# lalithsuresh/rapid

Hardware: NVIDIA H100
Metric: alert_cells_per_sec_to_converged_cut (higher is better)
Workload: dtype u16

## Files before the change

rapid_b200/csrc/cd_bucketed.cu:

```cuda
#include <cooperative_groups.h>

#include <algorithm>
#include <climits>
#include <cstdlib>

#include "cd_internal.cuh"

namespace cg = cooperative_groups;

namespace rapid {

constexpr int UNI_MINBLOCKS = 5;
constexpr int PF_DIST = 2;

constexpr int TILE_R = 1024;
constexpr int UNI_THREADS = 128;
constexpr int GEN_THREADS = 256;
constexpr int STAGE = 32;
constexpr int MAXK = RAPID_MAX_K;
constexpr int SMALL_SEG = 4;
constexpr uint32_t T32_NONE = 0xFFFFFFFFu;
constexpr uint64_t T64_NONE = ~0ULL;
constexpr uint32_t RF_K3 = 16u;
constexpr uint32_t RF_ACTIVE = 32u;
constexpr uint32_t RF_MIXED_EMIT = 64u;

constexpr uint32_t MX_ON = 1u, MX_NEG = 2u, MX_HAS_E = 4u, MX_DONE = 8u;
constexpr uint32_t MX_REF = 32u;
constexpr uint32_t MX_TIME = 16u;

constexpr uint32_t PF_SEEN = 1u;
constexpr uint32_t PF_NEGINF = 2u;

struct ChunkAcc {
    uint32_t nL, nH, tp, nUn, fl, minTH, minTLun, pad_;
    uint64_t h1, h2;
    uint32_t nLp, nHp, tpc, minBHp, minBLlong, pad2_;
    uint64_t h1p, h2p;
};

constexpr int PF_SHIFT = 30;
constexpr uint32_t TP_MASK = (1u << PF_SHIFT) - 1u;

struct Partials {
    uint4* cnt;
    uint4* cntp;
    uint64_t* minTH;
    uint64_t* minTLun;
    uint64_t* h1;
    uint64_t* h2;
    uint64_t* h1p;
    uint64_t* h2p;
    uint2* seq;
    int32_t* flag;
    ChunkAcc* chunk;
    int n_tiles;
};

struct Bucketed {
    DevBuf<int32_t> sidx;
    DevBuf<int32_t> seg_cnt, batch_slots;
    DevBuf<int32_t> bins, ovf, cell_batch;
    DevBuf<SubjDesc> desc;
    DevBuf<SubjWalk> walk;
    DevBuf<uint8_t> s_ring, s_status;
    DevBuf<int32_t> p_flag;
    DevBuf<ChunkAcc> p_chunk;
    DevBuf<uint4> p_cnt, p_cntp;
    DevBuf<uint64_t> p_minTH, p_minTLun, p_h1, p_h2, p_h1p, p_h2p;
    DevBuf<uint2> p_seq;
    DevBuf<SubjWalk> pwalk;
    DevBuf<unsigned char> ra_dev;
    DevBuf<uint32_t> mx_fl;
    DevBuf<uint64_t> mx_a, mx_cand, mx_emax;
    DevBuf<uint64_t> mx_p1, mx_p2;
    DevBuf<int32_t> mx_pc;
    DevBuf<unsigned long long> mx_e1, mx_e2;
    DevBuf<int32_t> mx_ec;
    DevBuf<uint64_t> estar;
    DevBuf<int32_t> mx_changed;
    DevBuf<uint32_t> mx_dev;
    DevBuf<int32_t> batch_index;
    DevBuf<int32_t> inv_res, inv_ticket;
    DevBuf<unsigned long long> inv_h1, inv_h2;
    DevBuf<int32_t> wl_slots, wl_count, wl_listed, wl_so_tab;
    DevBuf<uint8_t> wl_in_tile;
    DevBuf<uint8_t> has_so;
    size_t in_list_slots = 0;
    int n_tiles = 0;
    size_t part_cap = 0;
    int slots_uniform = 0, slots_generic = 0;
    int resolve_grid = 0;
};

struct Visit {
    int c0, c1;
    bool crossL, crossH;
    uint32_t tL, tH;
};

__device__ __forceinline__ Visit visit_uniform(uint32_t ur, const SubjDesc& d, const SubjWalk& w, int L, int H) {
    Visit v;
    v.tL = 0; v.tH = 0;
    if (ur == d.pmask) {
        v.c0 = __popc(ur); v.c1 = __popc(ur | d.bmask);
        v.tL = d.tLf; v.tH = d.tHf;
    } else {
        int c = __popc(ur);
        v.c0 = c;
        const int nr = d.nr;
        for (int q = 0; q < nr; ++q) {
            const int k = w.ring[q];
            const bool isnew = !((ur >> k) & 1u);
            c += isnew;
            if (isnew && c == L) v.tL = w.time[q];
            if (isnew && c == H) v.tH = w.time[q];
        }
        v.c1 = c;
    }
    v.crossL = v.c0 < L && v.c1 >= L;
    v.crossH = v.c0 < H && v.c1 >= H;
    return v;
}

__device__ __forceinline__ Visit visit_counts(uint32_t ur, const SubjDesc& d, uint32_t RM, int L, int H) {
    Visit v;
    v.tL = 0; v.tH = 0;
    v.c0 = __popc(ur);
    v.c1 = __popc((ur | d.bmask) & RM);
    v.crossL = v.c0 < L && v.c1 >= L;
    v.crossH = v.c0 < H && v.c1 >= H;
    return v;
}

struct Acc {
    uint32_t nL = 0, nH = 0, tp = 0, nUn = 0, flags = 0;
    uint32_t minTH = T32_NONE, minTLun = T32_NONE;
    uint64_t h1 = 0, h2 = 0;
    uint32_t nLp = 0, nHp = 0, tpc = 0, minBHp = T32_NONE, minBLlong = T32_NONE;
    uint64_t h1p = 0, h2p = 0;
};

__device__ __forceinline__ bool accumulate(Acc& a, const Visit& v, const SubjDesc& d, int L, int H) {
    if (v.c0 >= L && v.c0 < H) a.tp++;
    if (v.crossL) a.nL++;
    if (v.crossH) { a.nH++; a.minTH = min(a.minTH, v.tH); a.h1 += d.mix1; a.h2 += d.mix2; }
    if (v.c1 >= L && v.c1 < H) {
        if (v.crossL) { a.nUn++; a.minTLun = min(a.minTLun, v.tL); }
        else a.flags |= PF_NEGINF;
        return true;
    }
    return false;
}

__device__ __forceinline__ uint32_t prefix_core(Acc* acc, uint32_t ur, const SubjDesc& d, const SubjWalk& pw, const uint32_t* u,
                                                uint32_t umask, int L, int H, uint32_t last) {
    const int c0 = __popc(ur);
    int c = c0;
    uint32_t word = ur, bLp = 0, bHp = 0;
    if (ur == 0 && umask == 0) {
        c = __popc(d.pmask); bLp = d.f_bLp; bHp = d.f_bHp; word = d.pmask;
    } else {
        const int np = __popc(d.pmask);
        uint32_t imp = umask & ~ur;
        uint32_t bL = c >= L ? 0u : T32_NONE;
        int q = 0;
        for (;;) {
            while (q < np && ((word >> pw.ring[q]) & 1u)) ++q;
            const uint32_t te = q < np ? pw.time[q] : T32_NONE;
            uint32_t ti = T32_NONE;
            if (imp && c >= L && c < H) {
                for (uint32_t m = imp; m; m &= m - 1) { const int k = __ffs(m) - 1; if (u[k] != T32_NONE) ti = min(ti, max(u[k], bL)); }
                if (ti > last) ti = T32_NONE;
            }
            if (ti != T32_NONE && ti < te) {
                for (uint32_t m = imp; m; m &= m - 1) {
                    const int k = __ffs(m) - 1;
                    if (u[k] == T32_NONE || u[k] > ti) continue;
                    word |= 1u << k; imp &= ~(1u << k);
                    ++c;
                    if (c == H) bHp = ti;
                }
                if (c >= H) imp = 0;
            } else if (te != T32_NONE) {
                const int k = pw.ring[q];
                word |= 1u << k; imp &= ~(1u << k);
                ++c; ++q;
                if (c == L) { bL = te; bLp = te; }
                if (c == H) bHp = te;
            } else {
                break;
            }
        }
    }
    if (acc) {
        if (c0 >= L && c0 < H) acc->tpc++;
        if (c0 < L && c >= L) acc->nLp++;
        if (c0 < H && c >= H) { acc->nHp++; acc->h1p += d.mix1; acc->h2p += d.mix2; acc->minBHp = min(acc->minBHp, bHp); }
        if (c >= L && c < H) acc->minBLlong = min(acc->minBLlong, c0 >= L ? 0u : bLp);
    }
    return word;
}

__device__ __forceinline__ uint32_t observer_L_batch(uint32_t uo, const SubjDesc* dobs, const SubjWalk* pwo, int L) {
    int c = __popc(uo);
    if (c >= L) return 0u;
    if (dobs == nullptr || dobs->pmask == 0) return T32_NONE;
    const int np = __popc(dobs->pmask);
    for (int q = 0; q < np; ++q) {
        if ((uo >> pwo->ring[q]) & 1u) continue;
        if (++c == L) return pwo->time[q];
    }
    return T32_NONE;
}

struct ApplyArgs {
    RowRef rows;
    size_t Rpad;
    int K, H, L;
    int64_t R, rbegin;
    const uint32_t* rflags;
    DeliveryDev dl;
    const BatchCounts* bc;
    const SubjDesc* desc;
    const SubjWalk* walk;
    const SubjWalk* pwalk;
    const int32_t* touch;
    const int32_t* batch_index;
    int32_t serial;
    int seq;
    const int32_t* slot_subject;
    const int32_t* sidx;
    const uint8_t* s_ring;
    const uint8_t* s_status;
    Partials part;
    int n_tiles;
    WorkList wl;
};

__device__ __forceinline__ void note_unresolved(const ApplyArgs& a, int tile, int32_t slot) { worklist_note(a.wl, tile, slot); }

template <bool SEQ>
__device__ __forceinline__ void part_store(const Partials& p, size_t at, const Acc& a) {
    p.cnt[at] = make_uint4(a.nL, a.nH, a.tp | (a.flags << PF_SHIFT), a.nUn);
    if (SEQ) p.cntp[at] = make_uint4(a.nLp, a.nHp, a.tpc, 0u);
    p.minTH[at] = a.minTH == T32_NONE ? T64_NONE : (uint64_t)a.minTH;
    p.minTLun[at] = a.minTLun == T32_NONE ? T64_NONE : (uint64_t)a.minTLun;
    p.h1[at] = a.h1;
    p.h2[at] = a.h2;
    if (SEQ) { p.h1p[at] = a.h1p; p.h2p[at] = a.h2p; p.seq[at] = make_uint2(a.minBHp, a.minBLlong); }
}
template <bool SEQ>
__device__ __forceinline__ void part_merge(const Partials& p, size_t at, const Acc& a) {
    uint4 c = p.cnt[at];
    c.x += a.nL; c.y += a.nH; c.z = (c.z + a.tp) | (a.flags << PF_SHIFT); c.w += a.nUn;
    p.cnt[at] = c;
    if (SEQ && (a.nLp | a.nHp | a.tpc)) { uint4 cp = p.cntp[at]; cp.x += a.nLp; cp.y += a.nHp; cp.z += a.tpc; p.cntp[at] = cp; }
    if (a.minTH != T32_NONE) { const uint64_t o = p.minTH[at]; if ((uint64_t)a.minTH < o) p.minTH[at] = a.minTH; }
    if (a.minTLun != T32_NONE) { const uint64_t o = p.minTLun[at]; if ((uint64_t)a.minTLun < o) p.minTLun[at] = a.minTLun; }
    if (a.nH) { p.h1[at] += a.h1; p.h2[at] += a.h2; }
    if (SEQ) {
        if (a.nHp) { p.h1p[at] += a.h1p; p.h2p[at] += a.h2p; }
        uint2 q = p.seq[at];
        q.x = min(q.x, a.minBHp); q.y = min(q.y, a.minBLlong);
        p.seq[at] = q;
    }
}

struct StageAcc {
    uint32_t nLH, tpUn, fl, minTH, minTLun;
    uint64_t h1, h2;
    uint32_t nLHp, tpc, minBHp, minBLlong;
    uint64_t h1p, h2p;
};

template <bool SEQ>
__device__ __forceinline__ StageAcc stage_pack(const Acc& f) {
    StageAcc s;
    s.nLH = f.nL | (f.nH << 16); s.tpUn = f.tp | (f.nUn << 16); s.fl = f.flags; s.minTH = f.minTH; s.minTLun = f.minTLun;
    s.h1 = f.h1; s.h2 = f.h2;
    s.nLHp = SEQ ? f.nLp | (f.nHp << 16) : 0u; s.tpc = SEQ ? f.tpc : 0u; s.minBHp = SEQ ? f.minBHp : T32_NONE;
    s.minBLlong = SEQ ? f.minBLlong : T32_NONE; s.h1p = SEQ ? f.h1p : 0ull; s.h2p = SEQ ? f.h2p : 0ull;
    return s;
}
template <bool SEQ>
__device__ __forceinline__ StageAcc stage_reduce(StageAcc s) {
#pragma unroll
    for (int o = 16; o > 0; o >>= 1) {
        s.nLH += __shfl_down_sync(0xffffffffu, s.nLH, o);
        s.tpUn += __shfl_down_sync(0xffffffffu, s.tpUn, o);
        s.fl |= __shfl_down_sync(0xffffffffu, s.fl, o);
        s.minTH = min(s.minTH, __shfl_down_sync(0xffffffffu, s.minTH, o));
        s.minTLun = min(s.minTLun, __shfl_down_sync(0xffffffffu, s.minTLun, o));
        s.h1 += __shfl_down_sync(0xffffffffu, s.h1, o);
        s.h2 += __shfl_down_sync(0xffffffffu, s.h2, o);
        if (SEQ) {
            s.nLHp += __shfl_down_sync(0xffffffffu, s.nLHp, o);
            s.tpc += __shfl_down_sync(0xffffffffu, s.tpc, o);
            s.minBHp = min(s.minBHp, __shfl_down_sync(0xffffffffu, s.minBHp, o));
            s.minBLlong = min(s.minBLlong, __shfl_down_sync(0xffffffffu, s.minBLlong, o));
            s.h1p += __shfl_down_sync(0xffffffffu, s.h1p, o);
            s.h2p += __shfl_down_sync(0xffffffffu, s.h2p, o);
        }
    }
    return s;
}
template <bool SEQ>
__device__ __forceinline__ void chunk_add(ChunkAcc& c, const StageAcc& m) {
    c.nL += m.nLH & 0xFFFFu; c.nH += m.nLH >> 16; c.tp += m.tpUn & 0xFFFFu; c.nUn += m.tpUn >> 16; c.fl |= m.fl;
    c.minTH = min(c.minTH, m.minTH); c.minTLun = min(c.minTLun, m.minTLun); c.h1 += m.h1; c.h2 += m.h2;
    if (SEQ) {
        c.nLp += m.nLHp & 0xFFFFu; c.nHp += m.nLHp >> 16; c.tpc += m.tpc; c.minBHp = min(c.minBHp, m.minBHp);
        c.minBLlong = min(c.minBLlong, m.minBLlong); c.h1p += m.h1p; c.h2p += m.h2p;
    }
}
__device__ __forceinline__ ChunkAcc chunk_zero() {
    ChunkAcc c;
    c.nL = 0; c.nH = 0; c.tp = 0; c.nUn = 0; c.fl = 0; c.minTH = T32_NONE; c.minTLun = T32_NONE; c.pad_ = 0; c.h1 = 0; c.h2 = 0;
    c.nLp = 0; c.nHp = 0; c.tpc = 0; c.minBHp = T32_NONE; c.minBLlong = T32_NONE; c.pad2_ = 0; c.h1p = 0; c.h2p = 0;
    return c;
}
template <bool SEQ>
__device__ __forceinline__ void acc_add(Acc& a, const StageAcc& m) {
    a.nL += m.nLH & 0xFFFFu; a.nH += m.nLH >> 16; a.tp += m.tpUn & 0xFFFFu; a.nUn += m.tpUn >> 16; a.flags |= m.fl;
    a.minTH = min(a.minTH, m.minTH); a.minTLun = min(a.minTLun, m.minTLun); a.h1 += m.h1; a.h2 += m.h2;
    if (SEQ) {
        a.nLp += m.nLHp & 0xFFFFu; a.nHp += m.nLHp >> 16; a.tpc += m.tpc; a.minBHp = min(a.minBHp, m.minBHp);
        a.minBLlong = min(a.minBLlong, m.minBLlong); a.h1p += m.h1p; a.h2p += m.h2p;
    }
}

template <bool PERM, bool SEQ>
__device__ __forceinline__ bool visit_acc(Acc& acc, uint32_t ur, const SubjDesc& d, const SubjWalk* w, const SubjWalk* pw, uint32_t RM, int L, int H,
                                          const uint32_t* u = nullptr, uint32_t umask = 0, uint32_t last = 0, uint32_t* word_out = nullptr) {
    if (SEQ) ur = prefix_core(&acc, ur, d, *pw, u, umask, L, H, last);
    if (word_out) *word_out = ur;
    const Visit v = PERM ? visit_counts(ur & RM, d, RM, L, H) : visit_uniform(ur & RM, d, *w, L, H);
    return accumulate(acc, v, d, L, H);
}

constexpr uint32_t RF_PRE_DOWN = 128u;
__device__ __forceinline__ uint32_t receiver_down_batch(const ApplyArgs& a, uint32_t rflag, bool after_finalize1) {
    if (rflag & (after_finalize1 ? RF_PRE_DOWN : RF_SEEN_DOWN)) return 0u;
    const int32_t sd = a.bc->seq_down;
    return sd == INT_MAX ? T32_NONE : (uint32_t)sd;
}
__device__ __forceinline__ const uint8_t* precall_row(const ApplyArgs& a, int32_t slot, bool post_flip) {
    const int flipped = post_flip && a.touch[slot] == a.serial ? 1 : 0;
    return a.rows.lo(slot, a.rows.cur[slot] ^ flipped);
}
__device__ __noinline__ uint32_t edge_times(const ApplyArgs& a, int32_t slot, int64_t r, bool post_flip, uint32_t bDown, uint32_t* u) {
    if (!a.wl.has_so[slot]) return 0u;
    const uint32_t RM = (1u << a.K) - 1u;
    const int32_t S_before = a.bc->S_before;
    uint32_t umask = 0;
    for (int k = 0; k < a.K; ++k) {
        const int32_t so = a.wl.so_tab[(size_t)slot * SO_STRIDE + k];
        if (so < 0) continue;
        const bool ot = a.touch[so] == a.serial;
        const int bo = ot ? a.batch_index[so] : 0;
        const uint32_t uo = so >= S_before ? 0u : (a.rows.get(precall_row(a, so, post_flip), r) & RM);
        const uint32_t bLo = observer_L_batch(uo, ot ? &a.desc[bo] : nullptr, ot ? &a.pwalk[bo] : nullptr, a.L);
        u[k] = (bLo == T32_NONE || bDown == T32_NONE) ? T32_NONE : max(bLo, bDown);
        umask |= 1u << k;
    }
    return umask;
}
__device__ __forceinline__ uint32_t seq_state(const ApplyArgs& a, const SubjDesc& d, int b_index, int64_t r, uint32_t old, bool post_flip,
                                              bool after_finalize1) {
    if (!a.seq) return old;
    uint32_t u[MAXK];
    const uint32_t umask = edge_times(a, d.slot, r, post_flip, receiver_down_batch(a, a.rflags[r], after_finalize1), u);
    if (umask == 0 && d.pmask == 0) return old;
    return prefix_core(nullptr, old, d, a.pwalk[b_index], u, umask, a.L, a.H, (uint32_t)a.bc->seq_last);
}

template <bool PERM, bool SEQ, int HB>
__global__ void __launch_bounds__(UNI_THREADS, UNI_MINBLOCKS) k_apply_uniform(const ApplyArgs a) {
    __shared__ SubjDesc sd[STAGE];
    __shared__ SubjWalk sw[PERM ? 1 : STAGE];
    __shared__ SubjWalk spw[SEQ ? STAGE : 1];
    __shared__ const uint8_t* s_src[STAGE];
    __shared__ uint8_t* s_dst[STAGE];
    __shared__ uint32_t s_nw[STAGE];
    __shared__ uint2 s_nrep[STAGE];
    __shared__ int s_unres[STAGE];
    __shared__ ChunkAcc s_facc;
    __shared__ int s_heavy;
    __shared__ uint8_t s_ne[SEQ ? STAGE : 1];
    __shared__ uint8_t s_ek[SEQ ? STAGE : 1][MAXK];
    __shared__ const uint8_t* s_erow[SEQ ? STAGE : 1][MAXK];
    __shared__ int32_t s_eob[SEQ ? STAGE : 1][MAXK];
    __shared__ uint32_t s_mst[STAGE];
    __shared__ uint2 s_mrep[STAGE];
    __shared__ uint8_t s_mun[STAGE];
    __shared__ StageAcc s_macc[STAGE];
    __shared__ StageAcc s_msum;
    __shared__ uint32_t s_mall;
    __shared__ int s_wfirst[UNI_THREADS / 32];

    constexpr bool MEMO = !SEQ;
    if (a.bc->overflow) return;
    const int Sb = a.bc->n_batch_subj, S_before = a.bc->S_before;
    const int per_chunk = max(1, (Sb + (int)gridDim.y - 1) / (int)gridDim.y);
    const int tile = blockIdx.x, chunk = blockIdx.y, t = threadIdx.x;
    const int s0 = min(Sb, chunk * per_chunk), s1 = min(Sb, s0 + per_chunk);
    const int64_t r0 = (int64_t)tile * TILE_R + (int64_t)t * 8;
    const size_t pbase = (size_t)chunk * a.Rpad + (size_t)r0;
    const uint32_t RM = (1u << a.K) - 1u;
    const int L = a.L, H = a.H;
    const uint32_t seq_last = SEQ ? (uint32_t)a.bc->seq_last : 0u;

    uint32_t act = 0, seen = 0;
#pragma unroll
    for (int j = 0; j < 8; ++j) {
        const int64_t r = r0 + j;
        if (r < a.R) {
            const uint32_t rf = a.rflags[r];
            const bool on = !(rf & RF_ANNOUNCED) && !((a.dl.flags & RAPID_DELIVERY_BLOCKED) && a.dl.blocked[r]);
            act |= (on ? 1u : 0u) << j;
            if (SEQ && (rf & RF_SEEN_DOWN)) seen |= 1u << j;
        }
    }
    const Group8<HB> am = group8_mask<HB>(act);
    const RowRef& rows = a.rows;
    if (t == 0) s_facc = chunk_zero();
    if (MEMO) {
        const int mine = act ? t * 8 + __ffs(act) - 1 : INT_MAX;
        const int wmin = __reduce_min_sync(0xffffffffu, mine);
        if ((t & 31) == 0) s_wfirst[t >> 5] = wmin;
    }
    const int block_active = __syncthreads_or(act != 0);
    int sample_r = 0;
    if (MEMO && t < 32) {
        int f = INT_MAX;
#pragma unroll
        for (int q = 0; q < UNI_THREADS / 32; ++q) f = min(f, s_wfirst[q]);
        sample_r = f == INT_MAX ? 0 : f;
    }
    const size_t sample_at = (size_t)tile * TILE_R + (size_t)sample_r;
    Acc com;
    bool had_exc = false;
    bool carried = false;

    for (int base = s0; base < s1; base += STAGE) {
        const int n = min(STAGE, s1 - base);
        __syncthreads();
        if (t < 32) {
            Acc f;
            Acc m;
            bool heavy = false, memo = false;
            if (t < n) {
                const SubjDesc d = a.desc[base + t];
                sd[t] = d;
                const uint8_t c = rows.cur[d.slot];
                const bool fresh = d.slot >= S_before;
                s_src[t] = fresh ? nullptr : rows.lo(d.slot, c);
                s_dst[t] = rows.lo(d.slot, c ^ 1);
                s_nw[t] = (uint32_t)(d.bmask | d.pmask);
                s_nrep[t] = group8_rep<HB>(d.bmask | d.pmask);
                int un = 0;
                const bool edges = SEQ && a.wl.has_so[d.slot];
                if (SEQ) {
                    int ne = 0;
                    if (edges) {
                        for (int k = 0; k < a.K; ++k) {
                            const int32_t so = a.wl.so_tab[(size_t)d.slot * SO_STRIDE + k];
                            if (so < 0) continue;
                            s_ek[t][ne] = (uint8_t)k;
                            s_erow[t][ne] = so >= S_before ? nullptr : rows.cur_lo(so);
                            s_eob[t][ne] = a.touch[so] == a.serial ? a.batch_index[so] : -1;
                            ++ne;
                        }
                    }
                    s_ne[t] = (uint8_t)ne;
                }
                if (fresh && !edges) {
                    un = (visit_acc<PERM, SEQ>(f, 0u, d, &sw[0], &spw[0], RM, L, H) && block_active) ? 1 : 0;
                    if (PERM) { f.minTH = T32_NONE; f.minTLun = T32_NONE; }
                } else {
                    if (!PERM) sw[t] = a.walk[base + t];
                    if (SEQ) spw[t] = a.pwalk[base + t];
                    if (fresh) s_src[t] = nullptr;
                    if (MEMO && !fresh && !edges && block_active) {
                        const uint32_t sst = rows.get(s_src[t], (int64_t)sample_at);
                        uint32_t at_last = sst;
                        const bool mun = visit_acc<PERM, SEQ>(m, sst & RM, d, &sw[PERM ? 0 : t], &spw[SEQ ? t : 0], RM, L, H, nullptr, 0u, seq_last, &at_last);
                        s_mst[t] = sst;
                        s_mrep[t] = group8_rep<HB>((SEQ ? at_last : sst) | s_nw[t]);
                        s_mun[t] = mun ? 1 : 0;
                        memo = true;
                    }
                }
                if (MEMO) { if (!memo) s_mst[t] = 0xFFFFFFFFu; else s_macc[t] = stage_pack<SEQ>(m); }
                s_unres[t] = (un && a.wl.has_so[d.slot]) ? 1 : 0;
                if (!fresh || edges) s_unres[t] = a.wl.has_so[d.slot] ? 0 : -1;
                heavy = !fresh || edges;
            }
            {
                const unsigned hm = __ballot_sync(0xffffffffu, heavy);
                if (t == 0) s_heavy = __popc(hm);
            }
            const StageAcc fr = stage_reduce<SEQ>(stage_pack<SEQ>(f));
            if (t == 0) chunk_add<SEQ>(s_facc, fr);
            if (MEMO) {
                const unsigned mm = __ballot_sync(0xffffffffu, memo);
                if (mm) {
                    const StageAcc mr = stage_reduce<SEQ>(stage_pack<SEQ>(m));
                    if (t == 0) s_msum = mr;
                }
                if (t == 0) s_mall = mm;
            }
        }
        __syncthreads();
        uint32_t hit = 0;
        const bool pf_on = !SEQ && s_heavy != 0;
        if (pf_on) {
#pragma unroll
            for (int j = 0; j < PF_DIST; ++j)
                if (j < n && s_src[j]) {
                    asm volatile("prefetch.global.L2 [%0];" ::"l"(s_src[j] + r0));
                    asm volatile("prefetch.global.L2 [%0];" ::"l"(group8_hi<HB>(rows, s_src[j], r0)));
                }
        }
#pragma unroll 4
        for (int i = 0; i < n; ++i) {
            const uint8_t* src = s_src[i];
            uint8_t* dst = s_dst[i];
            const int ne = SEQ ? (int)s_ne[i] : 0;
            if (pf_on && i + PF_DIST < n) {
                const uint8_t* nx = s_src[i + PF_DIST];
                if (nx) {
                    asm volatile("prefetch.global.L2 [%0];" ::"l"(nx + r0));
                    asm volatile("prefetch.global.L2 [%0];" ::"l"(group8_hi<HB>(rows, nx, r0)));
                }
            }
            if (src == nullptr && ne == 0) {
                group8_store<HB>(rows, dst, r0, group8_fill<HB>(s_nrep[i], am));
                continue;
            }
            Group8<HB> w;
            if (src) w = group8_load<HB>(rows, src, r0);
            else { w.lo = 0; w.hi = 0; }
            bool unres = false;
            if (act) {
                const SubjDesc& d = sd[i];
                uint32_t st;
                bool same = group8_same<HB>(w, am, &st);
                carried = true;
                const bool mhit = MEMO && same && st == s_mst[i];
                uint32_t u[MAXK];
                uint32_t umask = 0;
                if (SEQ && ne && !mhit) {
                    const uint32_t sact = seen & act;
                    same = same && (sact == 0 || sact == act);
                    const uint32_t bDown = sact ? 0u : (a.bc->seq_down == INT_MAX ? T32_NONE : (uint32_t)a.bc->seq_down);
                    for (int e = 0; e < ne && same; ++e) {
                        uint32_t so_st = 0;
                        if (s_erow[i][e]) same = group8_same<HB>(group8_load<HB>(rows, s_erow[i][e], r0), am, &so_st);
                        const int ob = s_eob[i][e], k = s_ek[i][e];
                        const uint32_t bLo = observer_L_batch(so_st & RM, ob >= 0 ? &a.desc[ob] : nullptr, ob >= 0 ? &a.pwalk[ob] : nullptr, L);
                        u[k] = (bLo == T32_NONE || bDown == T32_NONE) ? T32_NONE : max(bLo, bDown);
                        umask |= 1u << k;
                    }
                }
                if (mhit) {
                    hit |= 1u << i;
                    unres = s_mun[i] != 0;
                    group8_merge<HB>(w, s_mrep[i], am);
                } else if (same) {
                    uint32_t at_last = st;
                    unres = visit_acc<PERM, SEQ>(com, st & RM, d, &sw[PERM ? 0 : i], &spw[SEQ ? i : 0], RM, L, H, u, umask, seq_last, &at_last);
                    group8_merge<HB>(w, group8_rep<HB>((SEQ ? at_last : st) | s_nw[i]), am);
                } else {
                    if (!had_exc) {
                        had_exc = true;
                        const Acc zero;
#pragma unroll
                        for (int j = 0; j < 8; ++j) part_store<SEQ>(a.part, pbase + j, zero);
                    }
                    const uint32_t nwb = s_nw[i];
#pragma unroll (SEQ ? 1 : 8)
                    for (int j = 0; j < 8; ++j) {
                        if (!((act >> j) & 1u)) continue;
                        const uint32_t sj = group8_word<HB>(w, j);
                        Acc ex;
                        uint32_t at_last = sj;
                        if (SEQ && ne) umask = edge_times(a, d.slot, r0 + j, false, receiver_down_batch(a, ((seen >> j) & 1u) ? RF_SEEN_DOWN : 0u, false), u);
                        unres |= visit_acc<PERM, SEQ>(ex, sj & RM, d, &sw[PERM ? 0 : i], &spw[SEQ ? i : 0], RM, L, H, u, umask, seq_last, &at_last);
                        part_merge<SEQ>(a.part, pbase + j, ex);
                        group8_or_word<HB>(w, j, (SEQ ? (at_last & RM) : 0u) | nwb);
                    }
                }
            }
            group8_store<HB>(rows, dst, r0, w);
            if (__any_sync(0xffffffffu, unres) && (t & 31) == 0 && s_unres[i] == 0) s_unres[i] = 1;
        }
        if (MEMO && hit) {
            if (hit == s_mall) acc_add<SEQ>(com, s_msum);
            else for (uint32_t mh = hit; mh; mh &= mh - 1) acc_add<SEQ>(com, s_macc[__ffs(mh) - 1]);
        }
        __syncthreads();
        if (t < n && s_unres[t] > 0) note_unresolved(a, tile, sd[t].slot);
    }
    const int need = __syncthreads_or((carried || had_exc) ? 1 : 0);
    if (t == 0) {
        a.part.flag[(size_t)chunk * a.part.n_tiles + tile] = need;
        if (tile == 0) a.part.chunk[chunk] = s_facc;
    }
    if (!need) return;
    const Acc zero;
#pragma unroll
    for (int j = 0; j < 8; ++j) {
        const size_t at = pbase + j;
        const bool on = (act >> j) & 1u;
        if (!had_exc) part_store<SEQ>(a.part, at, on ? com : zero);
        else if (on) part_merge<SEQ>(a.part, at, com);
    }
}

struct GVisit {
    int c0, c1;
    bool crossL, crossH, seen_down;
    uint64_t tL, tH;
    uint32_t have;
};

__device__ __forceinline__ GVisit visit_generic(uint32_t ur, const SubjDesc& d, const int32_t* __restrict__ sidx,
                                                const uint8_t* __restrict__ s_ring, const uint8_t* __restrict__ s_status,
                                                const DeliveryDev& dl, int64_t r, uint64_t rs, int L, int H) {
    GVisit v;
    v.have = 0; v.seen_down = false; v.tL = 0; v.tH = 0;
    const bool has_bitmap = dl.flags & RAPID_DELIVERY_BITMAP, permuted = dl.flags & RAPID_DELIVERY_PERMUTED;
    if (d.seg_len <= SMALL_SEG) {
        uint64_t tm[SMALL_SEG];
        int rk[SMALL_SEG];
        bool ok[SMALL_SEG];
#pragma unroll
        for (int j = 0; j < SMALL_SEG; ++j) {
            ok[j] = false; tm[j] = 0; rk[j] = 0;
            if (j < (int)d.seg_len) {
                const int32_t ci = sidx[d.seg_begin + j];
                if (!has_bitmap || ((dl.bitmap[(size_t)ci * dl.words + (r >> 5)] >> (r & 31)) & 1u)) {
                    ok[j] = true;
                    rk[j] = s_ring[d.seg_begin + j];
                    tm[j] = permuted ? splitmix64(rs ^ (uint64_t)(ci - dl.cell_base)) : (uint64_t)ci + 1ull;
                    if (s_status[d.seg_begin + j] == RAPID_EDGE_DOWN) v.seen_down = true;
                    v.have |= 1u << rk[j];
                }
            }
        }
        const uint32_t fresh = v.have & ~ur;
        v.c0 = __popc(ur);
        v.c1 = v.c0 + __popc(fresh);
        v.crossL = v.c0 < L && v.c1 >= L;
        v.crossH = v.c0 < H && v.c1 >= H;
        if (v.crossL || v.crossH) {
            const int wantL = L - v.c0 - 1, wantH = H - v.c0 - 1;
            bool first[SMALL_SEG];
#pragma unroll
            for (int j = 0; j < SMALL_SEG; ++j) {
                first[j] = ok[j] && !((ur >> rk[j]) & 1u);
#pragma unroll
                for (int i = 0; i < SMALL_SEG; ++i)
                    if (i != j && ok[i] && rk[i] == rk[j] && tm[i] < tm[j]) first[j] = false;
            }
#pragma unroll
            for (int j = 0; j < SMALL_SEG; ++j) {
                if (!first[j]) continue;
                int rank = 0;
#pragma unroll
                for (int i = 0; i < SMALL_SEG; ++i) rank += (first[i] && tm[i] < tm[j]) ? 1 : 0;
                if (rank == wantL) v.tL = tm[j];
                if (rank == wantH) v.tH = tm[j];
            }
        }
        return v;
    }
    uint64_t tmin[MAXK];
#pragma unroll
    for (int k = 0; k < MAXK; ++k) tmin[k] = 0;
    const uint32_t e = d.seg_begin + d.seg_len;
    for (uint32_t j = d.seg_begin; j < e; ++j) {
        const int32_t ci = sidx[j];
        if (has_bitmap && !((dl.bitmap[(size_t)ci * dl.words + (r >> 5)] >> (r & 31)) & 1u)) continue;
        if (s_status[j] == RAPID_EDGE_DOWN) v.seen_down = true;
        const int k = s_ring[j];
        const uint64_t tm = permuted ? splitmix64(rs ^ (uint64_t)(ci - dl.cell_base)) : (uint64_t)ci + 1ull;
        const bool had = (v.have >> k) & 1u;
#pragma unroll
        for (int kk = 0; kk < MAXK; ++kk)
            if (kk == k && (!had || tm < tmin[kk])) tmin[kk] = tm;
        v.have |= 1u << k;
    }
    const uint32_t fresh = v.have & ~ur;
    v.c0 = __popc(ur);
    v.c1 = v.c0 + __popc(fresh);
    v.crossL = v.c0 < L && v.c1 >= L;
    v.crossH = v.c0 < H && v.c1 >= H;
    if (v.crossL || v.crossH) {
        const int wantL = L - v.c0 - 1, wantH = H - v.c0 - 1;
#pragma unroll
        for (int k = 0; k < MAXK; ++k) {
            if (!((fresh >> k) & 1u)) continue;
            int rank = 0;
#pragma unroll
            for (int q = 0; q < MAXK; ++q) rank += (((fresh >> q) & 1u) && tmin[q] < tmin[k]) ? 1 : 0;
            if (rank == wantL) v.tL = tmin[k];
            if (rank == wantH) v.tH = tmin[k];
        }
    }
    return v;
}

__global__ void __launch_bounds__(GEN_THREADS, 4) k_apply_generic(const ApplyArgs a) {
    __shared__ SubjDesc sd[STAGE];
    __shared__ const uint8_t* s_src[STAGE];
    __shared__ uint8_t* s_dst[STAGE];
    __shared__ int s_unres[STAGE];
    if (a.bc->overflow) return;
    const int Sb = a.bc->n_batch_subj, S_before = a.bc->S_before;
    const int per_chunk = max(1, (Sb + (int)gridDim.y - 1) / (int)gridDim.y);
    const int t = threadIdx.x, chunk = blockIdx.y;
    const int64_t r = (int64_t)blockIdx.x * GEN_THREADS + t;
    const int tile = (int)(((int64_t)blockIdx.x * GEN_THREADS) / TILE_R);
    const int s0 = min(Sb, chunk * per_chunk), s1 = min(Sb, s0 + per_chunk);
    const uint32_t RM = (1u << a.K) - 1u;
    const int L = a.L, H = a.H;
    const bool in_range = r < a.R;
    const bool active = in_range && !(a.rflags[r] & RF_ANNOUNCED) && !((a.dl.flags & RAPID_DELIVERY_BLOCKED) && a.dl.blocked[r]);
    const uint64_t rs = splitmix64(a.dl.perm_seed + (uint64_t)(a.rbegin + r));
    uint32_t nL = 0, nH = 0, tp = 0, nUn = 0, fl = 0;
    uint64_t minTH = T64_NONE, minTLun = T64_NONE, h1 = 0, h2 = 0;
    bool haveTH = false, haveTL = false;
    for (int base = s0; base < s1; base += STAGE) {
        const int n = min(STAGE, s1 - base);
        __syncthreads();
        if (t < n) {
            const SubjDesc d = a.desc[base + t];
            sd[t] = d;
            const uint8_t c = a.rows.cur[d.slot];
            s_src[t] = d.slot >= S_before ? nullptr : a.rows.lo(d.slot, c);
            s_dst[t] = a.rows.lo(d.slot, c ^ 1);
            s_unres[t] = a.wl.has_so[d.slot] ? 0 : -1;
        }
        __syncthreads();
        uint32_t pre[8];
        for (int i = 0; i < n; ++i) {
            if ((i & 7) == 0) {
#pragma unroll
                for (int u = 0; u < 8; ++u) pre[u] = (i + u < n && s_src[i + u]) ? a.rows.get(s_src[i + u], r) : 0u;
            }
            const SubjDesc& d = sd[i];
            bool unres = false;
            if (r < (int64_t)a.Rpad) {
                uint32_t st = pre[i & 7];
                if (active) {
                    const GVisit v = visit_generic(st & RM, d, a.sidx, a.s_ring, a.s_status, a.dl, r, rs, L, H);
                    if (v.seen_down) fl |= PF_SEEN;
                    if (v.c0 >= L && v.c0 < H) tp++;
                    if (v.crossL) nL++;
                    if (v.crossH) {
                        nH++;
                        if (!haveTH || v.tH < minTH) { minTH = v.tH; haveTH = true; }
                        h1 += d.mix1; h2 += d.mix2;
                    }
                    if (v.c1 >= L && v.c1 < H) {
                        unres = true;
                        if (v.crossL) { nUn++; if (!haveTL || v.tL < minTLun) { minTLun = v.tL; haveTL = true; } }
                        else fl |= PF_NEGINF;
                    }
                    st |= v.have;
                }
                if (a.rows.hb == 2) row_store1_warp<2>(a.rows, s_dst[i], r, st);
                else row_store1_warp<8>(a.rows, s_dst[i], r, st);
            }
            if (__any_sync(0xffffffffu, unres) && (t & 31) == 0 && s_unres[i] == 0) s_unres[i] = 1;
        }
        __syncthreads();
        if (t < n && s_unres[t] > 0) note_unresolved(a, tile, sd[t].slot);
    }
    if (t == 0) {
        if ((blockIdx.x * GEN_THREADS) % TILE_R == 0) a.part.flag[(size_t)chunk * a.part.n_tiles + tile] = 1;
        if (blockIdx.x == 0) a.part.chunk[chunk] = chunk_zero();
    }
    if (r < (int64_t)a.Rpad) {
        const size_t p = (size_t)chunk * a.Rpad + (size_t)r;
        a.part.cnt[p] = make_uint4(nL, nH, tp | (fl << PF_SHIFT), nUn);
        a.part.minTH[p] = minTH;
        a.part.minTLun[p] = minTLun;
        a.part.h1[p] = h1;
        a.part.h2[p] = h2;
    }
}

struct ResolveArgs {
    ApplyArgs ap;
    MarkPlane emit;
    MarkPlane trans;
    BatchCounts* bc;
    BatchCounts* snap;
    int n_chunks;
    int uniform;
    int counts_only;
    int seq;
    uint8_t* seq_dev;
    uint8_t* cur_w;
    int32_t* n_pre;
    uint32_t* rflags;
    uint64_t* pend_h1;
    uint64_t* pend_h2;
    int32_t* pend_cnt;
    uint64_t* out_h1;
    uint64_t* out_h2;
    int32_t* out_len;
    uint8_t* out_ann;
    uint32_t* mx_fl;
    uint64_t* mx_a;
    uint64_t* mx_cand;
    uint64_t* mx_emax;
    uint64_t* mx_p1;
    uint64_t* mx_p2;
    int32_t* mx_pc;
    uint64_t* estar;
    unsigned long long* mx_e1;
    unsigned long long* mx_e2;
    int32_t* mx_ec;
    int32_t* mx_changed;
    uint32_t* mx_dev;
    const int32_t* slot_of;
    const int32_t* obs;
    const int32_t* touch;
    const int32_t* batch_index;
    int32_t serial;
    int inv_split;
    int32_t* inv_res;
    unsigned long long* inv_h1;
    unsigned long long* inv_h2;
    int32_t* inv_ticket;
};

__device__ __forceinline__ int32_t block_sum_i32(int32_t v, int32_t* s_red) {
    __syncthreads();
#pragma unroll
    for (int o = 16; o > 0; o >>= 1) v += __shfl_down_sync(0xffffffffu, v, o);
    if ((threadIdx.x & 31) == 0) s_red[threadIdx.x >> 5] = v;
    __syncthreads();
    int32_t s = 0;
    for (int w = 0; w < (int)(blockDim.x >> 5); ++w) s += s_red[w];
    return s;
}

__device__ __forceinline__ void reduce_fresh(const ResolveArgs& a, ChunkAcc* s_fresh, int* s_fhave) {
    const ApplyArgs& ap = a.ap;
    if (threadIdx.x < 32) {
        uint32_t nL = 0, nH = 0, tp = 0, nUn = 0, fl = 0, mTH = T32_NONE, mTL = T32_NONE;
        uint64_t h1 = 0, h2 = 0;
        uint32_t nLp = 0, nHp = 0, tpc = 0, mBH = T32_NONE, mBL = T32_NONE;
        uint64_t h1p = 0, h2p = 0;
        for (int c = threadIdx.x; c < a.n_chunks; c += 32) {
            const ChunkAcc k = ap.part.chunk[c];
            nL += k.nL; nH += k.nH; tp += k.tp; nUn += k.nUn; fl |= k.fl;
            if (k.nH) mTH = min(mTH, k.minTH);
            if (k.nUn) mTL = min(mTL, k.minTLun);
            h1 += k.h1; h2 += k.h2;
            if (a.seq) {
                nLp += k.nLp; nHp += k.nHp; tpc += k.tpc; mBH = min(mBH, k.minBHp); mBL = min(mBL, k.minBLlong);
                h1p += k.h1p; h2p += k.h2p;
            }
        }
#pragma unroll
        for (int o = 16; o > 0; o >>= 1) {
            nL += __shfl_down_sync(0xffffffffu, nL, o); nH += __shfl_down_sync(0xffffffffu, nH, o);
            tp += __shfl_down_sync(0xffffffffu, tp, o);
            nUn += __shfl_down_sync(0xffffffffu, nUn, o); fl |= __shfl_down_sync(0xffffffffu, fl, o);
            mTH = min(mTH, __shfl_down_sync(0xffffffffu, mTH, o)); mTL = min(mTL, __shfl_down_sync(0xffffffffu, mTL, o));
            h1 += __shfl_down_sync(0xffffffffu, h1, o); h2 += __shfl_down_sync(0xffffffffu, h2, o);
            nLp += __shfl_down_sync(0xffffffffu, nLp, o); nHp += __shfl_down_sync(0xffffffffu, nHp, o);
            tpc += __shfl_down_sync(0xffffffffu, tpc, o);
            mBH = min(mBH, __shfl_down_sync(0xffffffffu, mBH, o)); mBL = min(mBL, __shfl_down_sync(0xffffffffu, mBL, o));
            h1p += __shfl_down_sync(0xffffffffu, h1p, o); h2p += __shfl_down_sync(0xffffffffu, h2p, o);
        }
        if (threadIdx.x == 0) {
            ChunkAcc f;
            f.nL = nL; f.nH = nH; f.tp = tp; f.nUn = nUn; f.fl = fl; f.minTH = mTH; f.minTLun = mTL; f.pad_ = 0; f.h1 = h1; f.h2 = h2;
            f.nLp = nLp; f.nHp = nHp; f.tpc = tpc; f.minBHp = mBH; f.minBLlong = mBL; f.pad2_ = 0; f.h1p = h1p; f.h2p = h2p;
            *s_fresh = f;
            *s_fhave = (nH ? 1 : 0) | (nUn ? 2 : 0);
        }
    }
    __syncthreads();
}

__device__ void phase_finalize1(const ResolveArgs& a, int32_t* s_red) {
    const ApplyArgs& ap = a.ap;
    const int any_down = a.bc->any_down;
    __shared__ ChunkAcc s_fresh;
    __shared__ int s_fhave;
    reduce_fresh(a, &s_fresh, &s_fhave);
    int32_t my_mixed = 0, my_times = 0;
    for (int64_t r = (int64_t)blockIdx.x * blockDim.x + threadIdx.x; r < ap.R; r += (int64_t)gridDim.x * blockDim.x) {
        a.mx_fl[r] = 0;
        uint32_t flags = a.rflags[r] & ~(RF_ANN_NOW | RF_K3 | RF_ACTIVE | RF_PRE_DOWN);
// ... 976 lines not shown
```

Measured before the change: 20.79 million.

## Software-pipeline carried-row loads in non-SEQ apply kernel with deferred exception pass

Splits k_apply_uniform into a non-SEQ path that only walks carried (non-fresh) subjects through a small register queue of read-only loads plus a deeper L2 prefetch stream. Non-uniform groups are deferred to a separate exception pass after the main loop. Fresh-only stages skip loads entirely. The aim is to hide global-memory latency on the row-gather loop. In exchange it costs extra registers under the min-blocks launch bound, and the exception rows are loaded a second time.

Result: faster. 21.36 million (median of 6 runs) (+2.7%).

```diff
diff --git a/rapid_b200/csrc/cd_bucketed.cu b/rapid_b200/csrc/cd_bucketed.cu
--- a/rapid_b200/csrc/cd_bucketed.cu
+++ b/rapid_b200/csrc/cd_bucketed.cu
@@ -11,7 +11,8 @@
 namespace rapid {
 
 constexpr int UNI_MINBLOCKS = 5;
-constexpr int PF_DIST = 2;
+constexpr int ROW_DEPTH = 2;
+constexpr int PF_DIST = 8;
 
 constexpr int TILE_R = 1024;
 constexpr int UNI_THREADS = 128;
@@ -375,6 +376,16 @@
     return prefix_core(nullptr, old, d, a.pwalk[b_index], u, umask, a.L, a.H, (uint32_t)a.bc->seq_last);
 }
 
+template <int HB>
+__device__ __forceinline__ Group8<HB> group8_load_ro(const RowRef& rows, const uint8_t* l, int64_t r) {
+    using Hi = typename Group8<HB>::Hi;
+    using HiL = typename std::conditional<HB == 2, unsigned short, unsigned long long>::type;
+    Group8<HB> g;
+    g.lo = __ldg(reinterpret_cast<const unsigned long long*>(l + r));
+    g.hi = (Hi)__ldg(reinterpret_cast<const HiL*>(group8_hi<HB>(rows, l, r)));
+    return g;
+}
+
 template <bool PERM, bool SEQ, int HB>
 __global__ void __launch_bounds__(UNI_THREADS, UNI_MINBLOCKS) k_apply_uniform(const ApplyArgs a) {
     __shared__ SubjDesc sd[STAGE];
@@ -385,8 +396,8 @@
     __shared__ uint32_t s_nw[STAGE];
     __shared__ uint2 s_nrep[STAGE];
     __shared__ int s_unres[STAGE];
+    __shared__ uint32_t s_carr;
     __shared__ ChunkAcc s_facc;
-    __shared__ int s_heavy;
     __shared__ uint8_t s_ne[SEQ ? STAGE : 1];
     __shared__ uint8_t s_ek[SEQ ? STAGE : 1][MAXK];
     __shared__ const uint8_t* s_erow[SEQ ? STAGE : 1][MAXK];
@@ -439,6 +450,74 @@
         sample_r = f == INT_MAX ? 0 : f;
     }
     const size_t sample_at = (size_t)tile * TILE_R + (size_t)sample_r;
+
+    auto stage_in = [&](int base) {
+        const int n = min(STAGE, s1 - base);
+        Acc f;
+        Acc m;
+        bool carried_subj = false, memo = false;
+        if (t < n) {
+            const SubjDesc d = a.desc[base + t];
+            sd[t] = d;
+            const uint8_t c = rows.cur[d.slot];
+            const bool fresh = d.slot >= S_before;
+            s_src[t] = fresh ? nullptr : rows.lo(d.slot, c);
+            s_dst[t] = rows.lo(d.slot, c ^ 1);
+            s_nw[t] = (uint32_t)(d.bmask | d.pmask);
+            s_nrep[t] = group8_rep<HB>(d.bmask | d.pmask);
+            int un = 0;
+            const bool edges = SEQ && a.wl.has_so[d.slot];
+            if (SEQ) {
+                int ne = 0;
+                if (edges) {
+                    for (int k = 0; k < a.K; ++k) {
+                        const int32_t so = a.wl.so_tab[(size_t)d.slot * SO_STRIDE + k];
+                        if (so < 0) continue;
+                        s_ek[t][ne] = (uint8_t)k;
+                        s_erow[t][ne] = so >= S_before ? nullptr : rows.cur_lo(so);
+                        s_eob[t][ne] = a.touch[so] == a.serial ? a.batch_index[so] : -1;
+                        ++ne;
+                    }
+                }
+                s_ne[t] = (uint8_t)ne;
+            }
+            if (fresh && !edges) {
+                un = (visit_acc<PERM, SEQ>(f, 0u, d, &sw[0], &spw[0], RM, L, H) && block_active) ? 1 : 0;
+                if (PERM) { f.minTH = T32_NONE; f.minTLun = T32_NONE; }
+            } else {
+                if (!PERM) sw[t] = a.walk[base + t];
+                if (SEQ) spw[t] = a.pwalk[base + t];
+                if (MEMO && !fresh && !edges && block_active) {
+                    const uint32_t sst = rows.get(s_src[t], (int64_t)sample_at);
+                    uint32_t at_last = sst;
+                    const bool mun = visit_acc<PERM, SEQ>(m, sst & RM, d, &sw[PERM ? 0 : t], &spw[SEQ ? t : 0], RM, L, H, nullptr, 0u, seq_last, &at_last);
+                    s_mst[t] = sst;
+                    s_mrep[t] = group8_rep<HB>((SEQ ? at_last : sst) | s_nw[t]);
+                    s_mun[t] = mun ? 1 : 0;
+                    memo = true;
+                }
+            }
+            if (MEMO) { if (!memo) s_mst[t] = 0xFFFFFFFFu; else s_macc[t] = stage_pack<SEQ>(m); }
+            s_unres[t] = (un && a.wl.has_so[d.slot]) ? 1 : 0;
+            if (!fresh || edges) s_unres[t] = a.wl.has_so[d.slot] ? 0 : -1;
+            carried_subj = !fresh;
+        }
+        {
+            const unsigned cm = __ballot_sync(0xffffffffu, carried_subj);
+            if (t == 0) s_carr = cm;
+        }
+        const StageAcc fr = stage_reduce<SEQ>(stage_pack<SEQ>(f));
+        if (t == 0) chunk_add<SEQ>(s_facc, fr);
+        if (MEMO) {
+            const unsigned mm = __ballot_sync(0xffffffffu, memo);
+            if (mm) {
+                const StageAcc mr = stage_reduce<SEQ>(stage_pack<SEQ>(m));
+                if (t == 0) s_msum = mr;
+            }
+            if (t == 0) s_mall = mm;
+        }
+    };
+
     Acc com;
     bool had_exc = false;
     bool carried = false;
@@ -446,159 +525,156 @@
     for (int base = s0; base < s1; base += STAGE) {
         const int n = min(STAGE, s1 - base);
         __syncthreads();
-        if (t < 32) {
-            Acc f;
-            Acc m;
-            bool heavy = false, memo = false;
-            if (t < n) {
-                const SubjDesc d = a.desc[base + t];
-                sd[t] = d;
-                const uint8_t c = rows.cur[d.slot];
-                const bool fresh = d.slot >= S_before;
-                s_src[t] = fresh ? nullptr : rows.lo(d.slot, c);
-                s_dst[t] = rows.lo(d.slot, c ^ 1);
-                s_nw[t] = (uint32_t)(d.bmask | d.pmask);
-                s_nrep[t] = group8_rep<HB>(d.bmask | d.pmask);
-                int un = 0;
-                const bool edges = SEQ && a.wl.has_so[d.slot];
-                if (SEQ) {
-                    int ne = 0;
-                    if (edges) {
-                        for (int k = 0; k < a.K; ++k) {
-                            const int32_t so = a.wl.so_tab[(size_t)d.slot * SO_STRIDE + k];
-                            if (so < 0) continue;
-                            s_ek[t][ne] = (uint8_t)k;
-                            s_erow[t][ne] = so >= S_before ? nullptr : rows.cur_lo(so);
-                            s_eob[t][ne] = a.touch[so] == a.serial ? a.batch_index[so] : -1;
-                            ++ne;
+        if (t < 32) stage_in(base);
+        __syncthreads();
+        if (!SEQ) {
+            const uint32_t cm = s_carr;
+            uint32_t hit = 0;
+            uint32_t exc = 0;
+            if (cm == 0) {
+#pragma unroll 4
+                for (int i = 0; i < n; ++i) group8_store<HB>(rows, s_dst[i], r0, group8_fill<HB>(s_nrep[i], am));
+            } else {
+                uint32_t issue = cm;
+                uint32_t pfq = cm;
+                auto next_load = [&]() {
+                    const Group8<HB> g = group8_load_ro<HB>(rows, s_src[__ffs(issue) - 1], r0);
+                    issue &= issue - 1;
+                    return g;
+                };
+                auto next_prefetch = [&]() {
+                    const uint8_t* nx = s_src[__ffs(pfq) - 1];
+                    pfq &= pfq - 1;
+                    asm volatile("prefetch.global.L2 [%0];" ::"l"(nx + r0));
+                    asm volatile("prefetch.global.L2 [%0];" ::"l"(group8_hi<HB>(rows, nx, r0)));
+                };
+                Group8<HB> q[ROW_DEPTH];
+#pragma unroll
+                for (int d = 0; d < ROW_DEPTH; ++d)
+                    if (issue) { q[d] = next_load(); pfq &= pfq - 1; }
+#pragma unroll
+                for (int d = 0; d < PF_DIST; ++d)
+                    if (pfq) next_prefetch();
+                for (int i = 0; i < n; ++i) {
+                    uint8_t* dst = s_dst[i];
+                    if (!((cm >> i) & 1u)) {
+                        group8_store<HB>(rows, dst, r0, group8_fill<HB>(s_nrep[i], am));
+                        continue;
+                    }
+                    Group8<HB> w = q[0];
+#pragma unroll
+                    for (int d = 0; d + 1 < ROW_DEPTH; ++d) q[d] = q[d + 1];
+                    if (issue) q[ROW_DEPTH - 1] = next_load();
+                    if (pfq) next_prefetch();
+                    bool unres = false;
+                    if (act) {
+                        uint32_t st;
+                        const bool same = group8_same<HB>(w, am, &st);
+                        carried = true;
+                        if (same && st == s_mst[i]) {
+                            hit |= 1u << i;
+                            unres = s_mun[i] != 0;
+                            group8_merge<HB>(w, s_mrep[i], am);
+                        } else if (same) {
+                            unres = visit_acc<PERM, false>(com, st & RM, sd[i], &sw[PERM ? 0 : i], &spw[0], RM, L, H);
+                            group8_merge<HB>(w, group8_rep<HB>(st | s_nw[i]), am);
+                        } else {
+                            exc |= 1u << i;
                         }
                     }
-                    s_ne[t] = (uint8_t)ne;
+                    if (!((exc >> i) & 1u)) group8_store<HB>(rows, dst, r0, w);
+                    if (__any_sync(0xffffffffu, unres) && (t & 31) == 0 && s_unres[i] == 0) s_unres[i] = 1;
                 }
-                if (fresh && !edges) {
-                    un = (visit_acc<PERM, SEQ>(f, 0u, d, &sw[0], &spw[0], RM, L, H) && block_active) ? 1 : 0;
-                    if (PERM) { f.minTH = T32_NONE; f.minTLun = T32_NONE; }
-                } else {
-                    if (!PERM) sw[t] = a.walk[base + t];
-                    if (SEQ) spw[t] = a.pwalk[base + t];
-                    if (fresh) s_src[t] = nullptr;
-                    if (MEMO && !fresh && !edges && block_active) {
-                        const uint32_t sst = rows.get(s_src[t], (int64_t)sample_at);
-                        uint32_t at_last = sst;
-                        const bool mun = visit_acc<PERM, SEQ>(m, sst & RM, d, &sw[PERM ? 0 : t], &spw[SEQ ? t : 0], RM, L, H, nullptr, 0u, seq_last, &at_last);
-                        s_mst[t] = sst;
-                        s_mrep[t] = group8_rep<HB>((SEQ ? at_last : sst) | s_nw[t]);
-                        s_mun[t] = mun ? 1 : 0;
-                        memo = true;
+            }
+            for (uint32_t em = exc; em; em &= em - 1) {
+                const int i = __ffs(em) - 1;
+                Group8<HB> w = group8_load_ro<HB>(rows, s_src[i], r0);
+                if (!had_exc) {
+                    had_exc = true;
+                    const Acc zero;
+#pragma unroll
+                    for (int j = 0; j < 8; ++j) part_store<false>(a.part, pbase + j, zero);
+                }
+                const SubjDesc& d = sd[i];
+                const uint32_t nwb = s_nw[i];
+                bool unres = false;
+#pragma unroll
+                for (int j = 0; j < 8; ++j) {
+                    if (!((act >> j) & 1u)) continue;
+                    Acc ex;
+                    unres |= visit_acc<PERM, false>(ex, group8_word<HB>(w, j) & RM, d, &sw[PERM ? 0 : i], &spw[0], RM, L, H);
+                    part_merge<false>(a.part, pbase + j, ex);
+                    group8_or_word<HB>(w, j, nwb);
+                }
+                group8_store<HB>(rows, s_dst[i], r0, w);
+                if (unres && s_unres[i] == 0) s_unres[i] = 1;
+            }
+            if (hit) {
+                if (hit == s_mall) acc_add<false>(com, s_msum);
+                else for (uint32_t mh = hit; mh; mh &= mh - 1) acc_add<false>(com, s_macc[__ffs(mh) - 1]);
+            }
+        } else {
+#pragma unroll 4
+            for (int i = 0; i < n; ++i) {
+                const uint8_t* src = s_src[i];
+                uint8_t* dst = s_dst[i];
+                const int ne = (int)s_ne[i];
+                if (src == nullptr && ne == 0) {
+                    group8_store<HB>(rows, dst, r0, group8_fill<HB>(s_nrep[i], am));
+                    continue;
+                }
+                Group8<HB> w;
+                if (src) w = group8_load<HB>(rows, src, r0);
+                else { w.lo = 0; w.hi = 0; }
+                bool unres = false;
+                if (act) {
+                    const SubjDesc& d = sd[i];
+                    uint32_t st;
+                    bool same = group8_same<HB>(w, am, &st);
+                    carried = true;
+                    uint32_t u[MAXK];
+                    uint32_t umask = 0;
+                    if (ne) {
+                        const uint32_t sact = seen & act;
+                        same = same && (sact == 0 || sact == act);
+                        const uint32_t bDown = sact ? 0u : (a.bc->seq_down == INT_MAX ? T32_NONE : (uint32_t)a.bc->seq_down);
+                        for (int e = 0; e < ne && same; ++e) {
+                            uint32_t so_st = 0;
+                            if (s_erow[i][e]) same = group8_same<HB>(group8_load<HB>(rows, s_erow[i][e], r0), am, &so_st);
+                            const int ob = s_eob[i][e], k = s_ek[i][e];
+                            const uint32_t bLo = observer_L_batch(so_st & RM, ob >= 0 ? &a.desc[ob] : nullptr, ob >= 0 ? &a.pwalk[ob] : nullptr, L);
+                            u[k] = (bLo == T32_NONE || bDown == T32_NONE) ? T32_NONE : max(bLo, bDown);
+                            umask |= 1u << k;
+                        }
+                    }
+                    if (same) {
+                        uint32_t at_last = st;
+                        unres = visit_acc<PERM, SEQ>(com, st & RM, d, &sw[PERM ? 0 : i], &spw[i], RM, L, H, u, umask, seq_last, &at_last);
+                        group8_merge<HB>(w, group8_rep<HB>(at_last | s_nw[i]), am);
+                    } else {
+                        if (!had_exc) {
+                            had_exc = true;
+                            const Acc zero;
+#pragma unroll
+                            for (int j = 0; j < 8; ++j) part_store<SEQ>(a.part, pbase + j, zero);
+                        }
+                        const uint32_t nwb = s_nw[i];
+#pragma unroll 1
+                        for (int j = 0; j < 8; ++j) {
+                            if (!((act >> j) & 1u)) continue;
+                            const uint32_t sj = group8_word<HB>(w, j);
+                            Acc ex;
+                            uint32_t at_last = sj;
+                            if (ne) umask = edge_times(a, d.slot, r0 + j, false, receiver_down_batch(a, ((seen >> j) & 1u) ? RF_SEEN_DOWN : 0u, false), u);
+                            unres |= visit_acc<PERM, SEQ>(ex, sj & RM, d, &sw[PERM ? 0 : i], &spw[i], RM, L, H, u, umask, seq_last, &at_last);
+                            part_merge<SEQ>(a.part, pbase + j, ex);
+                            group8_or_word<HB>(w, j, (at_last & RM) | nwb);
+                        }
                     }
                 }
-                if (MEMO) { if (!memo) s_mst[t] = 0xFFFFFFFFu; else s_macc[t] = stage_pack<SEQ>(m); }
-                s_unres[t] = (un && a.wl.has_so[d.slot]) ? 1 : 0;
-                if (!fresh || edges) s_unres[t] = a.wl.has_so[d.slot] ? 0 : -1;
-                heavy = !fresh || edges;
-            }
-            {
-                const unsigned hm = __ballot_sync(0xffffffffu, heavy);
-                if (t == 0) s_heavy = __popc(hm);
-            }
-            const StageAcc fr = stage_reduce<SEQ>(stage_pack<SEQ>(f));
-            if (t == 0) chunk_add<SEQ>(s_facc, fr);
-            if (MEMO) {
-                const unsigned mm = __ballot_sync(0xffffffffu, memo);
-                if (mm) {
-                    const StageAcc mr = stage_reduce<SEQ>(stage_pack<SEQ>(m));
-                    if (t == 0) s_msum = mr;
-                }
-                if (t == 0) s_mall = mm;
-            }
-        }
-        __syncthreads();
-        uint32_t hit = 0;
-        const bool pf_on = !SEQ && s_heavy != 0;
-        if (pf_on) {
-#pragma unroll
-            for (int j = 0; j < PF_DIST; ++j)
-                if (j < n && s_src[j]) {
-                    asm volatile("prefetch.global.L2 [%0];" ::"l"(s_src[j] + r0));
-                    asm volatile("prefetch.global.L2 [%0];" ::"l"(group8_hi<HB>(rows, s_src[j], r0)));
-                }
-        }
-#pragma unroll 4
-        for (int i = 0; i < n; ++i) {
-            const uint8_t* src = s_src[i];
-            uint8_t* dst = s_dst[i];
-            const int ne = SEQ ? (int)s_ne[i] : 0;
-            if (pf_on && i + PF_DIST < n) {
-                const uint8_t* nx = s_src[i + PF_DIST];
-                if (nx) {
-                    asm volatile("prefetch.global.L2 [%0];" ::"l"(nx + r0));
-                    asm volatile("prefetch.global.L2 [%0];" ::"l"(group8_hi<HB>(rows, nx, r0)));
-                }
-            }
-            if (src == nullptr && ne == 0) {
-                group8_store<HB>(rows, dst, r0, group8_fill<HB>(s_nrep[i], am));
-                continue;
-            }
-            Group8<HB> w;
-            if (src) w = group8_load<HB>(rows, src, r0);
-            else { w.lo = 0; w.hi = 0; }
-            bool unres = false;
-            if (act) {
-                const SubjDesc& d = sd[i];
-                uint32_t st;
-                bool same = group8_same<HB>(w, am, &st);
-                carried = true;
-                const bool mhit = MEMO && same && st == s_mst[i];
-                uint32_t u[MAXK];
-                uint32_t umask = 0;
-                if (SEQ && ne && !mhit) {
-                    const uint32_t sact = seen & act;
-                    same = same && (sact == 0 || sact == act);
-                    const uint32_t bDown = sact ? 0u : (a.bc->seq_down == INT_MAX ? T32_NONE : (uint32_t)a.bc->seq_down);
-                    for (int e = 0; e < ne && same; ++e) {
-                        uint32_t so_st = 0;
-                        if (s_erow[i][e]) same = group8_same<HB>(group8_load<HB>(rows, s_erow[i][e], r0), am, &so_st);
-                        const int ob = s_eob[i][e], k = s_ek[i][e];
-                        const uint32_t bLo = observer_L_batch(so_st & RM, ob >= 0 ? &a.desc[ob] : nullptr, ob >= 0 ? &a.pwalk[ob] : nullptr, L);
-                        u[k] = (bLo == T32_NONE || bDown == T32_NONE) ? T32_NONE : max(bLo, bDown);
-                        umask |= 1u << k;
-                    }
-                }
-                if (mhit) {
-                    hit |= 1u << i;
-                    unres = s_mun[i] != 0;
-                    group8_merge<HB>(w, s_mrep[i], am);
-                } else if (same) {
-                    uint32_t at_last = st;
-                    unres = visit_acc<PERM, SEQ>(com, st & RM, d, &sw[PERM ? 0 : i], &spw[SEQ ? i : 0], RM, L, H, u, umask, seq_last, &at_last);
-                    group8_merge<HB>(w, group8_rep<HB>((SEQ ? at_last : st) | s_nw[i]), am);
-                } else {
-                    if (!had_exc) {
-                        had_exc = true;
-                        const Acc zero;
-#pragma unroll
-                        for (int j = 0; j < 8; ++j) part_store<SEQ>(a.part, pbase + j, zero);
-                    }
-                    const uint32_t nwb = s_nw[i];
-#pragma unroll (SEQ ? 1 : 8)
-                    for (int j = 0; j < 8; ++j) {
-                        if (!((act >> j) & 1u)) continue;
-                        const uint32_t sj = group8_word<HB>(w, j);
-                        Acc ex;
-                        uint32_t at_last = sj;
-                        if (SEQ && ne) umask = edge_times(a, d.slot, r0 + j, false, receiver_down_batch(a, ((seen >> j) & 1u) ? RF_SEEN_DOWN : 0u, false), u);
-                        unres |= visit_acc<PERM, SEQ>(ex, sj & RM, d, &sw[PERM ? 0 : i], &spw[SEQ ? i : 0], RM, L, H, u, umask, seq_last, &at_last);
-                        part_merge<SEQ>(a.part, pbase + j, ex);
-                        group8_or_word<HB>(w, j, (SEQ ? (at_last & RM) : 0u) | nwb);
-                    }
-                }
-            }
-            group8_store<HB>(rows, dst, r0, w);
-            if (__any_sync(0xffffffffu, unres) && (t & 31) == 0 && s_unres[i] == 0) s_unres[i] = 1;
-        }
-        if (MEMO && hit) {
-            if (hit == s_mall) acc_add<SEQ>(com, s_msum);
-            else for (uint32_t mh = hit; mh; mh &= mh - 1) acc_add<SEQ>(com, s_macc[__ffs(mh) - 1]);
+                group8_store<HB>(rows, dst, r0, w);
+                if (__any_sync(0xffffffffu, unres) && (t & 31) == 0 && s_unres[i] == 0) s_unres[i] = 1;
+            }
         }
         __syncthreads();
         if (t < n && s_unres[t] > 0) note_unresolved(a, tile, sd[t].slot);
```
